# LuchnikovI/Differentiable-quantum-circuit-cuda

Hardware: AMD Instinct MI355X
Metric: gate-applications/sec (fwd+bwd) at n qubits (higher is better)
Workload: dtype c64 (f32)

## Files before the change

### differentiable-quantum-circuit-cuda_amd/csrc/qdc.hip

```cpp
#include "qdc_circuit.hpp"
#include "qdc_primitives.hpp"
#include "qdc_spec.hpp"

namespace {
template <int R>
struct SpecCheckTwo {
  __device__ __forceinline__ void operator()(qdc::cx (&xf)[R], qdc::cx (&xb)[R], const qdc::SpecEnv& E) const {
    constexpr uint32_t z[32] = {};
    qdc::spec_xchg_imm<6, false>(xf, E, z, z);
    qdc::spec_xchg<6, false>(xb, E, z, z, z, z);
  }
};
template <int R, int TB>
struct SpecCheckOne {
  __device__ __forceinline__ void operator()(qdc::cx (&x)[R], const qdc::SpecEnv& E) const {
    constexpr uint32_t z[32] = {};
    qdc::spec_xchg_imm<TB, true>(x, E, z, z);
    qdc::spec_xchg<TB, true>(x, E, z, z, z, z);
  }
};
}
#define QDC_SPEC_CHECK(name, threads, pass)                                                       \
  __global__ __launch_bounds__(threads) void name(qdc::chunk* f, qdc::chunk* b, const qdc::fop* ops, \
                                                  const qdc::cx* mats, qdc::fgeo fg, uint32_t l0,    \
// ... 455 lines not shown
  qdc::Plan p;
  if (!qdc::plan_lane(n, (int)R, pos2, pos1, 2048u, (reduces & 1) != 0, p, 1, (reduces & 2) ? 10u : 6u))
    return 1;
  const qdc::lgeo& g = p.lg;
  const unsigned v[10] = {(unsigned)(p.ampk + 1), g.nlow, g.nf, g.f0, g.f1, g.m0, g.m1,
                          (unsigned)(g.units & 0xffffffffu), (unsigned)(g.units >> 32), g.it};
  for (int i = 0; i < 10; ++i) out[i] = v[i];
  return 0;
}

static const char* spec_program_for(unsigned tile_bits, const unsigned* kinds, const unsigned* t1,
                                    const unsigned* t2, const unsigned long long* deps, size_t n,
                                    std::string& name, std::string& src) {
  if (n == 0 || n > 64) return "invalid arguments";
  std::vector<qdc::RqStage> st(n);
  for (size_t i = 0; i < n; ++i) st[i] = qdc::RqStage{kinds[i], t1[i], t2[i], deps ? deps[i] : 0};
  const bool force_one = (tile_bits & 0x100u) != 0, pf = (tile_bits & 0x200u) != 0;
  const bool spec_half = !(tile_bits & 0x400u);
  tile_bits &= 0xffu;
  const unsigned t2bits = sizeof(qdc::real) == 4 ? 11u : 10u;
  if (tile_bits != t2bits && tile_bits != t2bits + 1) return "tile_bits: not a specialized pass's tile";
  const bool two = tile_bits == t2bits && !force_one;
  qdc::RqKnobs knobs;
  if (tile_bits == t2bits && force_one) knobs.rq_wave |= pf ? 2 | 8 : 2;
  const qdc::RqVariant* V = qdc::rq_select(two, tile_bits, knobs, false);
  if (!V || !V->prefix) return "tile_bits: not a specialized pass's tile";
  const bool keep = spec_half && V->ns == 5;
  const qdc::RqPlan plan = qdc::rq_plan(st, tile_bits, nullptr, true, V->ns, keep);
  std::vector<qdc::SpecStep> sst;
  qdc::RqLayout cur = plan.load;
  for (const qdc::RqStep& s : plan.steps) {
    qdc::fop F{};
    if (s.relayout) {
      F.kind = qdc::FK_RELAYOUT;
      sst.push_back(qdc::SpecStep{true, cur, s.L, F});
      cur = s.L;
      continue;
    }
    F.kind = st[s.stage].kind | (two ? qdc::FOP_GAMMA : 0u);
    F.t1 = s.cs;
    const uint32_t kd = st[s.stage].kind;
    if ((kd == qdc::FK_Q2 || kd == qdc::FK_DIAG) && (s.cs >> 3) > (s.cs & 7u))
      F.t1 = (s.cs & 7u) * 8u + (s.cs >> 3);
    sst.push_back(qdc::SpecStep{false, cur, cur, F});
  }
  const bool half = V->pass_half && spec_half && !qdc::spec_imm() && qdc::spec_half_ok(sst);
  const qdc::SpecKind K = qdc::spec_kind(*V, half);
  const std::string body = qdc::spec_program_source(sst, tile_bits, K);
  name = qdc::spec_kernel_name(body, K);
  src = qdc::spec_kernel_source(name, body, K);
  return nullptr;
}

QDC_API const char* qdc_spec_selftest(unsigned tile_bits, const unsigned* kinds, const unsigned* t1,
// ... 240 lines not shown
```

### differentiable-quantum-circuit-cuda_amd/csrc/qdc_circuit.hpp

```cpp
#pragma once

#include <algorithm>
#include <cstring>
#include <memory>
#include <vector>

#include <rccl/rccl.h>

#include "qdc/circuit.h"
#include "qdc_device.hpp"
#include "qdc_shard.hpp"
#include "qdc_stage.hpp"
#include "qdc_fusion.hpp"
#include "qdc_jit.hpp"

namespace qdc {

struct Flat {
  const qdc_complex* data;
  std::vector<size_t> off;
  std::vector<size_t> len;
  Flat(const qdc_complex* d, const size_t* lens, size_t n) : data(d), off(n), len(n) {
    size_t o = 0;
    for (size_t i = 0; i < n; ++i) {
// ... 208 lines not shown
  int spec_async = sizeof(real) == 4 ? 1 : 0;
  std::map<std::vector<uint32_t>, SpecEntry> spec_cache;
  uint64_t spec_epoch = 0;
  int rq_permute = 1;
  int rq_perm_shard = 1;
  int rq_grad32 = 1;
  int rq_maxcl = 1;
  uint32_t rq_perm_low = 0;
  int rq_gstage = 1;
  uint32_t tile1_chunks = TILE_CHUNKS_1;
  int diag_inject = 1;
  int early_inject = 1;
  int dens1_kernel = 1;
  int dens_split = 1;
  int mirror = 1;
  int spec_half = 1;
  int defer_q1 = 1;
  bool mirror_on() const {
    return mirror && fuse && fuse_max_ops >= 2 && use_rq && (sizeof(real) == 4 || rq64);
  }
  const char* rq_variant(bool two, uint32_t tbits, const RqVariant*& V) const {
    V = rq_select(two, tbits, rqk, mirror_on());
    if (!V)
      return fail("no register-resident kernel for a %u-amplitude %s tile", 1u << tbits,
                  two ? "two-state" : "one-state");
    return nullptr;
  }
  bool rq_keep(const RqVariant& V) const { return spec_half && V.ns == 5; }

  bool dry = false;
  std::vector<unsigned char> dry_prog;
  std::vector<SpecEntry*> dry_specs;
  struct TraceOp {
    uint32_t dir, item, q2, q1, R, diag, mirrored, single;
    qdc_complex m[16];
  };
  bool tracing = false;
  std::vector<TraceOp> trace;
  size_t trace_from = 0;
  std::vector<uint8_t> inexact;
  uint32_t fused_blocks = 0;
  std::vector<std::pair<const void*, uint32_t>> fused_resident_cache;
  uint32_t last_fused_grid = 0;
  uint32_t last_fused_ndyn = 0;
  unsigned char* prog_host = nullptr;
  std::vector<StagePost> stage_post;
  size_t prog_cap = 0;

  Ctx& ctx0() { return devs[0]->ctx; }
  const char* sync_all() {
// ... 71 lines not shown
    if (const char* e = getenv("QDC_RW")) rqk.rq_wave = atoi(e);
    if (const char* e = getenv("QDC_RQ_ORDER")) rq_order = atoi(e);
    if (const char* e = getenv("QDC_RQ64")) rq64 = atoi(e);
    if (const char* e = getenv("QDC_RQ_SLOTS5")) rqk.rq_slots5 = atoi(e);
    if (const char* e = getenv("QDC_RQ_PERM")) rq_permute = atoi(e);
    if (const char* e = getenv("QDC_RQ_PERM_SHARD")) rq_perm_shard = atoi(e);
    if (const char* e = getenv("QDC_RQ_GRAD32")) rq_grad32 = atoi(e);
    if (const char* e = getenv("QDC_RQ_MAXCL")) rq_maxcl = atoi(e);
    if (const char* e = getenv("QDC_RQ_PERM_LOW")) rq_perm_low = (uint32_t)atoi(e);
    if (const char* e = getenv("QDC_RQ_GSTAGE")) rq_gstage = atoi(e);
    if (const char* e = getenv("QDC_DIAG_INJECT")) diag_inject = atoi(e);
    if (const char* e = getenv("QDC_EARLY_INJECT")) early_inject = atoi(e);
    if (const char* e = getenv("QDC_DENS1")) dens1_kernel = atoi(e);
    if (const char* e = getenv("QDC_DENS_SPLIT")) dens_split = atoi(e);
    if (const char* e = getenv("QDC_MIRROR")) mirror = atoi(e);
    if (const char* e = getenv("QDC_SPEC_HALF")) spec_half = atoi(e);
    if (const char* e = getenv("QDC_DEFER_Q1")) defer_q1 = atoi(e);
    if (const char* e = getenv("QDC_SCHED_CACHE")) sched_cache_on = atoi(e);
    if (const char* e = getenv("QDC_TILE1_CHUNKS")) {
      const uint32_t t = (uint32_t)atoi(e);
      if (t != TILE_CHUNKS_1 && t != TILE_CHUNKS_2)
        return fail("QDC_TILE1_CHUNKS must be %u or %u", TILE_CHUNKS_1, TILE_CHUNKS_2);
      tile1_chunks = t;
    }
    if (const char* e = getenv("QDC_SPEC")) spec_mode = atoi(e);
    if (const char* e = getenv("QDC_SPEC_MIN_QUBITS")) spec_min_qubits = (uint32_t)atoi(e);
    if (const char* e = getenv("QDC_SPEC_MAX")) spec_max = (uint32_t)atoi(e);
    if (const char* e = getenv("QDC_SPEC_FWD")) spec_fwd = atoi(e);
    if (const char* e = getenv("QDC_SPEC_ASYNC")) spec_async = atoi(e);
    SpecJit::get().set_processes(std::max(1, world / std::max(1, nlocal)));
// ... 692 lines not shown
      }
      g.diag = M.diag;
      g.role = stage_role(R, is_q1_gate(in.kind), op.pos2, lo, hi);
      const bool grad = two && is_var(in.kind);
      g.var = grad ? (int)B.var_idx[op.instr] : -1;
      any_grad = any_grad || grad;
    }
    SMat A;
    SMatD Bp;
    StagePost post;
    stage_compose(B.gates.data(), B.gates.size(), R, A, Bp, post);
    const bool all_diag = post.diag_only;
    if (rec_mats) (*rec_mats)[ii].push_back(A);
    SMat Aup = A;
    const bool from_fwd = B.backward && mirror_adjoint(B.plan, it, sj, R, Aup);
    if (tracing) {
      TraceOp t{B.backward ? 1u : 0u, (uint32_t)ii, hi, lo, (uint32_t)R, all_diag ? 1u : 0u,
                from_fwd ? 1u : 0u, 0u, {}};
      for (int i = 0; i < R * R; ++i) {
        const bool keep = !all_diag || i % (R + 1) == 0;
        t.m[i].re = keep ? (qdc_real)(real)Aup.a[i].real() : 0;
        t.m[i].im = keep ? (qdc_real)(real)Aup.a[i].imag() : 0;
      }
      trace.push_back(t);
    }
    fop& F = B.ops.back().F;
    F.t1 = local_bit(it, lo);
    F.t2 = local_bit(it, hi);
    F.mat = (uint32_t)B.mo;
    F.kind = (all_diag ? FK_DIAG : (R == 2 ? FK_Q1 : FK_Q2)) | (any_grad ? FOP_GAMMA : 0u);
    it.writes_f = true;
    const int nm = all_diag ? 4 : R * R;
    cx* m = B.mats + B.mo;
    for (int i = 0; i < nm; ++i) {
      const cd va = all_diag ? Aup.a[i * 4 + i] : Aup.a[i];
      const cdd vb = all_diag ? Bp.a[i * 4 + i] : Bp.a[i];
      m[i] = cx{(real)va.real(), (real)va.imag()};
      m[nm + i] = cx{(real)vb.real(), (real)vb.imag()};
    }
    B.mo += 2 * nm;
    const double cmac = all_diag ? 1.0 : (R == 2 ? 2.0 : 4.0);
    it.flops_per_amp += 8.0 * cmac * ((two ? 2.0 : 1.0) + (any_grad ? 1.0 : 0.0));
    if (any_grad) {
      post.slot = B.next_slot++;
      it.grad_slots.push_back(post.slot);
      B.ops.back().slot = (int)post.slot;
      it.has_red = true;
      stage_post.push_back(std::move(post));
    }
    return nullptr;
  }
  bool mirror_adjoint(const std::vector<qdc_plan_op>& plan, const Item& it, size_t sj, int R,
                      SMat& Aup) const {
    if (it.mirror_of.empty()) return false;
// ... 758 lines not shown
```

### differentiable-quantum-circuit-cuda_amd/csrc/qdc_jit.hpp

```cpp
#pragma once

#include <dirent.h>
#include <dlfcn.h>
#include <fcntl.h>
#include <spawn.h>
#include <sys/file.h>
#include <sys/stat.h>
#include <sys/wait.h>
#include <unistd.h>

#include <algorithm>
#include <atomic>
#include <chrono>
#include <cerrno>
#include <condition_variable>
#include <csignal>
#include <cstdlib>
#include <deque>
#include <ctime>
#include <cstdio>
#include <cstring>
#include <map>
#include <mutex>
#include <set>
// ... 128 lines not shown
    if (s.relayout) {
      const rq_layout c = rq_descriptor(s.Lc, T), n = rq_descriptor(s.Ln, T);
      b += "    { constexpr uint32_t rc[" + nr + "] = " + arr(c.rp, NR) + ", tc[8] = " + arr(c.tv, 8) +
           ", rn[" + nr + "] = " + arr(n.rp, NR) + ", tn[8] = " + arr(n.tv, 8) + ";\n      ";
      b += K.two ? "spec_xchg" + xt + "(xf, E, rc, tc, rn, tn); spec_xchg" + xt + "(xb, E, rc, tc, rn, tn); }\n"
                 : "spec_xchg" + xt + "(x, E, rc, tc, rn, tn); }\n";
      continue;
    }
    const uint32_t kind = s.F.kind & 7u;
    const bool gamma = K.two && (s.F.kind & FOP_GAMMA) != 0 && !(QDC_RQ_ABL & 4);
    const uint32_t c = s.F.t1;
    std::string tpl = kind == FK_Q1 ? "rq_q1<" + std::to_string(c)
                                    : std::string(kind == FK_DIAG ? "rq_diag<" : "rq_q2<") +
                                          std::to_string(c >> 3) + ", " + std::to_string(c & 7u);
    if (K.two)
      snprintf(tmp, sizeof tmp, "    %s, true, %u>(xf, xb, E.mats + E.ops[%zu].mat, %s, &E.accw[%u][0]);\n",
               tpl.c_str(), NR, j, gamma ? "true" : "false", ri);
    else
      snprintf(tmp, sizeof tmp, "    %s, false, %u>(x, x, E.mats + E.ops[%zu].mat, false, nullptr);\n",
               tpl.c_str(), NR, j);
    b += tmp;
    if (gamma) ++ri;
  }
  return b;
}
inline std::string spec_kernel_source(const std::string& name, const std::string& body, const SpecKind& K) {
  const std::string R = std::to_string(1u << K.ns);
  const std::string args =
      K.two ? "qdc::cx (&xf)[" + R + "], qdc::cx (&xb)[" + R + "], const qdc::SpecEnv& E"
            : "qdc::cx (&x)[" + R + "], const qdc::SpecEnv& E";
  return "#define QDC_SPEC_TU 1\n#include \"qdc_spec.hpp\"\n"
         "namespace {\n"
// ... 701 lines not shown
```

### differentiable-quantum-circuit-cuda_amd/csrc/qdc_kernels.hpp

```cpp
#pragma once

#include <cstddef>

#include <hip/hip_runtime.h>
#include <stdint.h>

#include <type_traits>

namespace qdc {

#ifdef QDC_F64
using real = double;
typedef double vec16 __attribute__((ext_vector_type(2)));
#else
using real = float;
typedef float vec16 __attribute__((ext_vector_type(4)));
#endif

struct cx {
  real x, y;
};

constexpr int VEC = 16 / (int)sizeof(cx);
constexpr int LV = (VEC == 2) ? 1 : 0;
// ... 971 lines not shown
#if QDC_PK_ASM
__device__ __forceinline__ pk2 pk_re_fma(pk2 a, pk2 f, pk2 c) {
  asm("v_pk_fma_f32 %0, %1, %2, %0 op_sel_hi:[0,1,1]" : "+v"(c) : "s"(a), "v"(f));
  return c;
}
__device__ __forceinline__ pk2 pk_im_fma(pk2 a, pk2 f, pk2 c) {
  asm("v_pk_fma_f32 %0, %1, %2, %0 op_sel:[1,1,0] op_sel_hi:[1,0,1] neg_lo:[1,0,0]"
      : "+v"(c) : "s"(a), "v"(f));
  return c;
}
__device__ __forceinline__ pk2 pk_re_mul(pk2 a, pk2 f) {
  pk2 r;
  asm("v_pk_mul_f32 %0, %1, %2 op_sel_hi:[0,1]" : "=v"(r) : "s"(a), "v"(f));
  return r;
}
#else
__device__ __forceinline__ pk2 pk_re_fma(pk2 a, pk2 f, pk2 c) {
  return __builtin_elementwise_fma(__builtin_shufflevector(a, a, 0, 0), f, c);
}
__device__ __forceinline__ pk2 pk_im_fma(pk2 a, pk2 f, pk2 c) {
  const pk2 na = -a;
  return __builtin_elementwise_fma(__builtin_shufflevector(na, a, 1, 3),
                                   __builtin_shufflevector(f, f, 1, 0), c);
}
__device__ __forceinline__ pk2 pk_re_mul(pk2 a, pk2 f) {
  return __builtin_shufflevector(a, a, 0, 0) * f;
}
#endif
#if QDC_PK_ASM || QDC_PK_VASM
__device__ __forceinline__ pk2 vpk_re_fma(pk2 a, pk2 f, pk2 c) {
  asm("v_pk_fma_f32 %0, %1, %2, %0 op_sel_hi:[0,1,1]" : "+v"(c) : "v"(a), "v"(f));
  return c;
}
__device__ __forceinline__ pk2 vpk_im_fma(pk2 a, pk2 f, pk2 c) {
  asm("v_pk_fma_f32 %0, %1, %2, %0 op_sel:[1,1,0] op_sel_hi:[1,0,1] neg_lo:[1,0,0]"
      : "+v"(c) : "v"(a), "v"(f));
  return c;
}
__device__ __forceinline__ pk2 vpk_re_mul(pk2 a, pk2 f) {
  pk2 r;
  asm("v_pk_mul_f32 %0, %1, %2 op_sel_hi:[0,1]" : "=v"(r) : "v"(a), "v"(f));
  return r;
}
#else
__device__ __forceinline__ pk2 vpk_re_fma(pk2 a, pk2 f, pk2 c) { return pk_re_fma(a, f, c); }
__device__ __forceinline__ pk2 vpk_im_fma(pk2 a, pk2 f, pk2 c) { return pk_im_fma(a, f, c); }
__device__ __forceinline__ pk2 vpk_re_mul(pk2 a, pk2 f) { return pk_re_mul(a, f); }
#endif
__device__ __forceinline__ cx ucfma(cx a, cx f, cx c) {
  const pk2 A = __builtin_bit_cast(pk2, a), F = __builtin_bit_cast(pk2, f);
  return __builtin_bit_cast(cx, pk_im_fma(A, F, pk_re_fma(A, F, __builtin_bit_cast(pk2, c))));
}
__device__ __forceinline__ cx ucmul(cx a, cx f) {
  const pk2 A = __builtin_bit_cast(pk2, a), F = __builtin_bit_cast(pk2, f);
  return __builtin_bit_cast(cx, pk_im_fma(A, F, pk_re_mul(A, F)));
}
__device__ __forceinline__ cx vcfma(cx a, cx f, cx c) {
  const pk2 A = __builtin_bit_cast(pk2, a), F = __builtin_bit_cast(pk2, f);
  return __builtin_bit_cast(cx, vpk_im_fma(A, F, vpk_re_fma(A, F, __builtin_bit_cast(pk2, c))));
}
__device__ __forceinline__ cx vcmul(cx a, cx f) {
  const pk2 A = __builtin_bit_cast(pk2, a), F = __builtin_bit_cast(pk2, f);
  return __builtin_bit_cast(cx, vpk_im_fma(A, F, vpk_re_mul(A, F)));
}
#else
__device__ __forceinline__ cx ucfma(cx a, cx f, cx c) { return cfma(a, f, c); }
__device__ __forceinline__ cx ucmul(cx a, cx f) { return cmul(a, f); }
__device__ __forceinline__ cx vcfma(cx a, cx f, cx c) { return cfma(a, f, c); }
__device__ __forceinline__ cx vcmul(cx a, cx f) { return cmul(a, f); }
#endif

template <int R>
__device__ __forceinline__ void umatvec(const cx* M, cx (&x)[R]) {
  cx y[R];
#pragma unroll
  for (int p = 0; p < R; ++p) {
    cx t = ucmul(M[p * R], x[0]);
#pragma unroll
    for (int q = 1; q < R; ++q) t = ucfma(M[p * R + q], x[q], t);
    y[p] = t;
  }
#pragma unroll
  for (int p = 0; p < R; ++p) x[p] = y[p];
}
// ... 13 lines not shown
      }
#pragma unroll
    for (int p = 0; p < R; ++p)
#pragma unroll
      for (int n = 0; n < NQ; ++n)
        y[n][p] = pk_im_fma(__builtin_bit_cast(pk2, M[p * R + q]), __builtin_bit_cast(pk2, x[n][q]),
                            y[n][p]);
  }
#pragma unroll
  for (int n = 0; n < NQ; ++n)
#pragma unroll
    for (int p = 0; p < R; ++p) x[n][p] = __builtin_bit_cast(cx, y[n][p]);
#else
#pragma unroll
  for (int n = 0; n < NQ; ++n) umatvec<R>(M, x[n]);
#endif
}

__device__ __forceinline__ uint32_t lane_sel(uint32_t f, uint32_t t, uint64_t mask) {
  uint32_t r;
  asm volatile("v_cndmask_b32_e64 %0, %1, %2, %3" : "=v"(r) : "v"(f), "v"(t), "s"(mask));
  return r;
}
__device__ __forceinline__ float lane_sel(float f, float t, uint64_t mask) {
  return __uint_as_float(lane_sel(__float_as_uint(f), __float_as_uint(t), mask));
}
__device__ __forceinline__ double lane_sel(double f, double t, uint64_t mask) {
  const uint64_t fb = (uint64_t)__double_as_longlong(f), tb = (uint64_t)__double_as_longlong(t);
  const uint64_t lo = lane_sel((uint32_t)fb, (uint32_t)tb, mask);
  const uint64_t hi = lane_sel((uint32_t)(fb >> 32), (uint32_t)(tb >> 32), mask);
// ... 123 lines not shown
__host__ __device__ __forceinline__ uint32_t swz(uint32_t i) {
  return i ^ (((i >> (4 + LV)) & 15u) << LV);
}
__device__ __forceinline__ uint32_t swz_chunk(uint32_t c) { return c ^ ((c >> 4) & 15u); }

enum : uint32_t {
  FK_Q1 = 0,
  FK_Q2 = 1,
  FK_DIAG = 2,
  FK_DENS1 = 3,
  FK_DENS2 = 4,
  FK_INJ1 = 5,
  FK_INJ2 = 6,
};
constexpr uint32_t FOP_GAMMA = 8;

#ifndef QDC_FUSED_WAVES
#define QDC_FUSED_WAVES 4
#endif
template <bool TWO, int TB, bool HASRED, bool WF, int NT>
__global__ __launch_bounds__(NT) __attribute__((amdgpu_waves_per_eu(NT == 256 ? QDC_FUSED_WAVES : 2)))
void k_fused(chunk* __restrict__ f, chunk* __restrict__ b, const fop* __restrict__ ops,
             const cx* __restrict__ mats, fgeo fg, cx* __restrict__ partials,
             uint64_t slot_stride) {
  constexpr int NS = TWO ? 2 : 1;
  constexpr int CPT = TB / NT;
  static_assert(TB % NT == 0 && TB * VEC >= 4 * NT, "tile must cover the block");
  __shared__ chunk lds[NS][TB];
  __shared__ real accw[HASRED ? NT / 64 : 1][HASRED ? FMAX_GRAD : 1][FACC];
  const uint32_t t = threadIdx.x;
// ... 529 lines not shown
```

### differentiable-quantum-circuit-cuda_amd/csrc/qdc_rq.hpp

```cpp
#pragma once

#include <type_traits>

#include "qdc_kernels.hpp"

namespace qdc {

#ifndef QDC_RQ_GSPLIT
#define QDC_RQ_GSPLIT 0
#endif
#ifndef QDC_MATVEC_N
#define QDC_MATVEC_N 1
#endif

constexpr int RQ_R = 16;
constexpr uint32_t FK_RELAYOUT = 7;
constexpr int RQ_NT_ONE = 256;
constexpr int RQ_NT_TWO = 128;

struct rq_layout {
  uint32_t rp[2 * RQ_R];
  uint32_t tv[8];
};
static_assert(sizeof(rq_layout) == 160 && sizeof(rq_layout) % sizeof(cx) == 0,
// ... 8 lines not shown
template <int S1, int S2>
__device__ __forceinline__ constexpr int rq_el(int base, int r) {
  return base | ((r & 1) << S1) | ((r >> 1) << S2);
}
template <int S1, int S2>
__device__ __forceinline__ constexpr int rq_base(int k) {
  int b = 0, bit = 0;
  for (int s = 0; s < 8; ++s) {
    if (s == S1 || s == S2) continue;
    if ((k >> bit) & 1) b |= 1 << s;
    ++bit;
  }
  return b;
}

template <int S1, int S2, bool TWO, int R>
__device__ __forceinline__ void rq_q2(cx (&f)[R], cx (&b)[R], const cx* __restrict__ M,
                                      bool gamma, real* acc_out) {
  cx A[16], B[16];
  if (TWO && gamma) {
    constexpr int NH = (QDC_RQ_GSPLIT && R >= 32) ? 2 : 1;
#pragma unroll
    for (int h = 0; h < NH; ++h) {
      constexpr int PR = 4 / NH;
      cx acc[4 * PR];
#pragma unroll
      for (int k = 0; k < R / 4; ++k) {
        const int base = rq_base<S1, S2>(k);
#pragma unroll
        for (int pp = 0; pp < PR; ++pp)
#pragma unroll
          for (int q = 0; q < 4; ++q) {
            const int p = h * PR + pp;
            const cx bp = b[rq_el<S1, S2>(base, p)], fq = f[rq_el<S1, S2>(base, q)];
            acc[pp * 4 + q] = k == 0 ? vcmul(bp, fq) : vcfma(bp, fq, acc[pp * 4 + q]);
          }
      }
      real v[8 * PR];
#pragma unroll
      for (int i = 0; i < 4 * PR; ++i) {
        v[2 * i] = acc[i].x;
        v[2 * i + 1] = acc[i].y;
      }
      wave_reduce_add<8 * PR>(v, acc_out + h * 8 * PR);
    }
  }
#pragma unroll
  for (int i = 0; i < 16; ++i) A[i] = M[i];
  constexpr int NQ = (QDC_MATVEC_N && R / 4 >= 2) ? 2 : 1;
#pragma unroll
  for (int k = 0; k < R / 4; k += NQ) {
    cx x[NQ][4];
#pragma unroll
    for (int n = 0; n < NQ; ++n)
#pragma unroll
      for (int r = 0; r < 4; ++r) x[n][r] = f[rq_el<S1, S2>(rq_base<S1, S2>(k + n), r)];
    umatvec_n<4, NQ>(A, x);
#pragma unroll
    for (int n = 0; n < NQ; ++n)
#pragma unroll
      for (int r = 0; r < 4; ++r) f[rq_el<S1, S2>(rq_base<S1, S2>(k + n), r)] = x[n][r];
  }
  if constexpr (TWO) {
#pragma unroll
// ... 2 lines not shown
    for (int k = 0; k < R / 4; k += NQ) {
      cx x[NQ][4];
#pragma unroll
      for (int n = 0; n < NQ; ++n)
#pragma unroll
        for (int r = 0; r < 4; ++r) x[n][r] = b[rq_el<S1, S2>(rq_base<S1, S2>(k + n), r)];
      umatvec_n<4, NQ>(B, x);
#pragma unroll
      for (int n = 0; n < NQ; ++n)
#pragma unroll
        for (int r = 0; r < 4; ++r) b[rq_el<S1, S2>(rq_base<S1, S2>(k + n), r)] = x[n][r];
    }
  }
}

template <int S1, int S2, bool TWO, int R>
__device__ __forceinline__ void rq_diag(cx (&f)[R], cx (&b)[R], const cx* __restrict__ M,
                                        bool gamma, real* acc_out) {
  cx A[4], B[4];
#pragma unroll
  for (int i = 0; i < 4; ++i) A[i] = M[i];
  if constexpr (TWO) {
#pragma unroll
    for (int i = 0; i < 4; ++i) B[i] = M[4 + i];
  }
  if (TWO && gamma) {
    cx acc[4];
#pragma unroll
    for (int k = 0; k < R / 4; ++k) {
      const int base = rq_base<S1, S2>(k);
#pragma unroll
      for (int r = 0; r < 4; ++r) {
        const int e = rq_el<S1, S2>(base, r);
        acc[r] = k == 0 ? vcmul(b[e], f[e]) : vcfma(b[e], f[e], acc[r]);
      }
    }
    real v[8];
#pragma unroll
    for (int i = 0; i < 4; ++i) {
      v[2 * i] = acc[i].x;
      v[2 * i + 1] = acc[i].y;
    }
    wave_reduce_add<8>(v, acc_out);
  }
#pragma unroll
  for (int k = 0; k < R / 4; ++k) {
    const int base = rq_base<S1, S2>(k);
#pragma unroll
    for (int r = 0; r < 4; ++r) {
      const int e = rq_el<S1, S2>(base, r);
      f[e] = ucmul(A[r], f[e]);
      if constexpr (TWO) b[e] = ucmul(B[r], b[e]);
    }
  }
}

template <int S, bool TWO, int R>
__device__ __forceinline__ void rq_q1(cx (&f)[R], cx (&b)[R], const cx* __restrict__ M,
                                      bool gamma, real* acc_out) {
  cx A[4], B[4];
#pragma unroll
  for (int i = 0; i < 4; ++i) A[i] = M[i];
  if constexpr (TWO) {
#pragma unroll
    for (int i = 0; i < 4; ++i) B[i] = M[4 + i];
  }
  constexpr int LOWM = (1 << S) - 1;
  if (TWO && gamma) {
    cx acc[4];
#pragma unroll
    for (int k = 0; k < R / 2; ++k) {
      const int j0 = ((k & ~LOWM) << 1) | (k & LOWM), j1 = j0 | (1 << S);
      const cx bx[2] = {b[j0], b[j1]}, fx[2] = {f[j0], f[j1]};
#pragma unroll
      for (int p = 0; p < 2; ++p)
#pragma unroll
        for (int q = 0; q < 2; ++q)
          acc[p * 2 + q] = k == 0 ? vcmul(bx[p], fx[q]) : vcfma(bx[p], fx[q], acc[p * 2 + q]);
    }
    real v[8];
#pragma unroll
    for (int i = 0; i < 4; ++i) {
      v[2 * i] = acc[i].x;
      v[2 * i + 1] = acc[i].y;
    }
    wave_reduce_add<8>(v, acc_out);
  }
  constexpr int NP = (QDC_MATVEC_N && R / 2 >= 4) ? 4 : 1;
#pragma unroll
  for (int k = 0; k < R / 2; k += NP) {
    cx x[NP][2];
#pragma unroll
    for (int n = 0; n < NP; ++n) {
      const int j0 = (((k + n) & ~LOWM) << 1) | ((k + n) & LOWM), j1 = j0 | (1 << S);
      x[n][0] = f[j0];
      x[n][1] = f[j1];
    }
    umatvec_n<2, NP>(A, x);
#pragma unroll
    for (int n = 0; n < NP; ++n) {
      const int j0 = (((k + n) & ~LOWM) << 1) | ((k + n) & LOWM), j1 = j0 | (1 << S);
      f[j0] = x[n][0];
      f[j1] = x[n][1];
    }
    if constexpr (TWO) {
#pragma unroll
      for (int n = 0; n < NP; ++n) {
        const int j0 = (((k + n) & ~LOWM) << 1) | ((k + n) & LOWM), j1 = j0 | (1 << S);
        x[n][0] = b[j0];
        x[n][1] = b[j1];
      }
      umatvec_n<2, NP>(B, x);
#pragma unroll
      for (int n = 0; n < NP; ++n) {
        const int j0 = (((k + n) & ~LOWM) << 1) | ((k + n) & LOWM), j1 = j0 | (1 << S);
        b[j0] = x[n][0];
        b[j1] = x[n][1];
      }
    }
  }
}

template <bool TWO, int R>
__device__ __forceinline__ void rq_stage(uint32_t sel, cx (&xf)[R], cx (&xb)[R],
                                         const cx* __restrict__ M, bool gamma, real* acc) {
#define QDC_RQ_Q2(S1, S2)                                                             \
  case FK_Q2 * 64 + (S1) * 8 + (S2):                                                  \
    if constexpr ((S2) < 4 || R >= 32) rq_q2<S1, S2, TWO, R>(xf, xb, M, gamma, acc);   \
    break;                                                                            \
  case FK_DIAG * 64 + (S1) * 8 + (S2):                                                \
    if constexpr ((S2) < 4 || R >= 32) rq_diag<S1, S2, TWO, R>(xf, xb, M, gamma, acc); \
    break;
  switch (sel) {
    QDC_RQ_Q2(0, 1) QDC_RQ_Q2(0, 2) QDC_RQ_Q2(0, 3) QDC_RQ_Q2(1, 2) QDC_RQ_Q2(1, 3)
    QDC_RQ_Q2(2, 3) QDC_RQ_Q2(0, 4) QDC_RQ_Q2(1, 4) QDC_RQ_Q2(2, 4) QDC_RQ_Q2(3, 4)
    case FK_Q1 * 64 + 0: rq_q1<0, TWO, R>(xf, xb, M, gamma, acc); break;
    case FK_Q1 * 64 + 1: rq_q1<1, TWO, R>(xf, xb, M, gamma, acc); break;
    case FK_Q1 * 64 + 2: rq_q1<2, TWO, R>(xf, xb, M, gamma, acc); break;
    case FK_Q1 * 64 + 4:
      if constexpr (R >= 32) rq_q1<4, TWO, R>(xf, xb, M, gamma, acc);
      break;
    default: rq_q1<3, TWO, R>(xf, xb, M, gamma, acc); break;
  }
#undef QDC_RQ_Q2
}

template <int LOGNT>
__device__ __forceinline__ uint32_t rq_tp(const rq_layout* L, uint32_t t) {
  uint32_t tp = 0;
#pragma unroll
  for (int k = 0; k < LOGNT; ++k) tp ^= ((t >> k) & 1u) ? L->tv[k] : 0u;
  return tp;
}

__device__ __forceinline__ void rq_exchange(cx (&x)[RQ_R], cx* buf, uint32_t tp,
                                            const rq_layout* Lc, uint32_t tpn,
                                            const rq_layout* Ln) {
#if !(QDC_RQ_ABL & 16)
  __syncthreads();
// ... 241 lines not shown
      }
      if ((QDC_RQ_ABL & 1) && kind != FK_RELAYOUT) {
        if (TWO && (op.kind & FOP_GAMMA)) ++ri;
        continue;
      }
      if (kind == FK_RELAYOUT) {
        const rq_layout* Lc = reinterpret_cast<const rq_layout*>(mats + lcur);
        const rq_layout* Ln = reinterpret_cast<const rq_layout*>(M);
        const uint32_t tp = TWO ? rq_tp<LOGNT>(Lc, t) : tpc, tpn = rq_tp<LOGNT>(Ln, t);
        rq_exchange(xf, buf, tp, Lc, tpn, Ln);
        if constexpr (TWO) rq_exchange(xb, buf, tp, Lc, tpn, Ln);
        tpc = tpn;
        lcur = op.mat;
        continue;
      }
      rq_stage<TWO>(kind * 64u + op.t1, xf, xb, M, gamma, acc);
      if (gamma) ++ri;
    }
  };
  if constexpr (!PF) {
    cx xf[RQ_R], xb[RQ_R];
    for (uint32_t tt = 0; tt < count; ++tt) {
      const uint64_t base = tile_base(tile0 + tt * tstep);
      load(xf, xb, base);
      run(xf, xb);
      store(xf, xb, base);
    }
  } else {
    static_assert(!TWO, "k_rq prefetch: one-state passes (qdc_variant.hpp)");
    constexpr int NLD = TWO ? 2 * CPT : CPT;
    vec16 pf_f[CPT];
// ... 254 lines not shown
        continue;
      }
      if ((QDC_RQ_ABL & 1) && kind != FK_RELAYOUT) {
        if (TWO && (op.kind & FOP_GAMMA)) ++ri;
        continue;
      }
      if (kind == FK_RELAYOUT) {
        const rq_layout* Lc = reinterpret_cast<const rq_layout*>(mats + lcur);
        const rq_layout* Ln = reinterpret_cast<const rq_layout*>(M);
        const uint32_t tp = rq_tp<TB>(Lc, lane), tpn = rq_tp<TB>(Ln, lane);
        exchange(xf, tp, Lc, tpn, Ln);
        if constexpr (TWO) exchange(xb, tp, Lc, tpn, Ln);
        lcur = op.mat;
        continue;
      }
      rq_stage<TWO>(kind * 64u + op.t1, xf, xb, M, gamma, acc);
      if (gamma) ++ri;
    }
  };
  auto flush_acc = [&](cx* dst, uint64_t stride) __attribute__((always_inline)) {
    __builtin_amdgcn_wave_barrier();
    for (uint32_t i = lane; i < fg.ngrad * FACC; i += 64) {
      const uint32_t k = i / FACC, e = i % FACC;
      reinterpret_cast<real*>(dst + (uint64_t)k * stride)[e] = accw[k][e];
      accw[k][e] = 0;
    }
    __builtin_amdgcn_wave_barrier();
  };
  cx xf[R], xb[R];
  if constexpr (!PF) {
    if (QDC_RQ_ABL & 32) {
// ... 182 lines not shown
```

### differentiable-quantum-circuit-cuda_amd/quantum_differentiable_circuit/__init__.py

```python
from __future__ import annotations

import ctypes as C
from typing import List, Sequence

import numpy as np

from .common_gates import get_cnot, get_hadamard
from ._native import (PanicException, KernelStat, PlanOp, check, default_precision, load,
                      ptr, PRECISIONS)
from .observable import PauliSum

__all__ = ["Circuit", "Circuit32", "Circuit64", "QuantizedTensor", "PanicException",
           "get_q1_grad", "get_q2_grad", "get_q2_grad_diag", "get_qk_grad", "data_transfer",
           "PauliSum", "pauli_inject",
           "circuit_class",
           "plan", "unpermute", "get_hadamard", "get_cnot"]

(CONST_Q2, VAR_Q2, CONST_Q2_NONU, VAR_Q2_NONU, CONST_Q2_DIAG, VAR_Q2_DIAG, CONST_Q1,
 CONST_Q1_NONU, VAR_Q1, VAR_Q1_NONU, Q2_DENSITY, Q1_DENSITY, DIFF_Q2_DENSITY,
 DIFF_Q1_DENSITY) = range(14)
MODE_RUN, MODE_FORWARD = 0, 1


def _array1(x, dtype, what):
# ... 414 lines not shown
    dens = [_array2(g, dt, "grads_wrt_density") for g in grads_wrt_density]
    df, dl = _flatten(dens, dt, "grads_wrt_density", "Gradient is not contiguous.")
    count = C.c_size_t(0)
    check(lib.qdc_precompile(int(qubits_number), int(world), kinds, a, b, m, ptr(cf), ptr(cl),
                             len(const_gates), ptr(vf), ptr(vl), len(var_gates), ptr(df), ptr(dl),
                             len(dens), C.byref(count)))
    return int(count.value)


def trace_program(qubits_number, instructions, const_gates, var_gates, grads_wrt_density,
                  world=1, precision=None):
    prec = precision or default_precision()
    lib = load(prec)
    dt = np.dtype(PRECISIONS[prec])
    rec = np.dtype([("dir", "<u4"), ("item", "<u4"), ("q2", "<u4"), ("q1", "<u4"), ("R", "<u4"),
                    ("diag", "<u4"), ("mirrored", "<u4"), ("single", "<u4"), ("m", dt, 16)])
    m = len(instructions)
    kinds = (C.c_int * m)(*[int(i[0]) for i in instructions])
    a = (C.c_uint * m)(*[int(i[1]) for i in instructions])
    b = (C.c_uint * m)(*[int(i[2]) if len(i) > 2 else 0 for i in instructions])
    cf, cl = _flat_gates(const_gates, dt, "const_gates")
    vf, vl = _flat_gates(var_gates, dt, "var_gates")
    dens = [_array2(g, dt, "grads_wrt_density") for g in grads_wrt_density]
    df, dl = _flatten(dens, dt, "grads_wrt_density", "Gradient is not contiguous.")
    cap = 4 * m + 64
    while True:
        out = np.zeros(cap, dtype=rec)
        cnt = C.c_size_t(0)
        check(lib.qdc_trace_program(int(qubits_number), int(world), kinds, a, b, m, ptr(cf),
                                    ptr(cl), len(const_gates), ptr(vf), ptr(vl), len(var_gates),
                                    ptr(df), ptr(dl), len(dens), ptr(out), cap, C.byref(cnt)))
# ... 245 lines not shown
```

### include/qdc/circuit.h

```cpp
#ifndef QDC_CIRCUIT_H
#define QDC_CIRCUIT_H

#include <stddef.h>

#include "qdc/primitives.h"

#ifdef __cplusplus
extern "C" {
#endif

enum qdc_kind {
  QDC_CONST_Q2 = 0,
  QDC_VAR_Q2 = 1,
  QDC_CONST_Q2_NONU = 2,
  QDC_VAR_Q2_NONU = 3,
  QDC_CONST_Q2_DIAG = 4,
  QDC_VAR_Q2_DIAG = 5,
  QDC_CONST_Q1 = 6,
  QDC_CONST_Q1_NONU = 7,
  QDC_VAR_Q1 = 8,
  QDC_VAR_Q1_NONU = 9,
  QDC_Q2_DENSITY = 10,
  QDC_Q1_DENSITY = 11,
  QDC_DIFF_Q2_DENSITY = 12,
// ... 122 lines not shown

const char* qdc_precompile(size_t qubits_number, int world, const int* kinds,
                           const unsigned* pos2, const unsigned* pos1, size_t count,
                           const qdc_complex* const_gates, const size_t* const_lens, size_t n_const,
                           const qdc_complex* var_gates, const size_t* var_lens, size_t n_var,
                           const qdc_complex* dens_grads, const size_t* dens_lens, size_t n_dens,
                           size_t* kernels);

const char* qdc_check_schedule(size_t qubits_number, int world, const int* kinds,
                               const unsigned* pos2, const unsigned* pos1, size_t count,
                               size_t* items, size_t* swaps);

typedef struct qdc_trace_op {
  unsigned dir, item, q2, q1, R, diag, mirrored, single;
  qdc_complex m[16];
} qdc_trace_op;

const char* qdc_trace_program(size_t qubits_number, int world, const int* kinds,
                              const unsigned* pos2, const unsigned* pos1, size_t count,
                              const qdc_complex* const_gates, const size_t* const_lens,
                              size_t n_const, const qdc_complex* var_gates,
                              const size_t* var_lens, size_t n_var, const qdc_complex* dens_grads,
                              const size_t* dens_lens, size_t n_dens, qdc_trace_op* out, size_t cap,
                              size_t* n_out);

#ifdef __cplusplus
}
#endif

#endif
// ... 1 lines not shown
```

Baseline: 4790.

## Derive backward-state gate matrix as conjugate of forward matrix in register kernels

For backward-pass fused gates whose instructions are unitary and exactly representable, the second (b) matrix is now set to the elementwise conjugate of the forward matrix. The register-resident kernels then load only the A matrix and apply it to both the forward and backward amplitudes, using packed FMA variants that negate the imaginary part. This saves matrix loads and registers. Matrix fetches are also moved ahead of the gradient reduction, with a scheduling barrier, so their latency overlaps that work; a LATE flag keeps the old fetch order when the feature is disabled. The trace format grows to expose the b matrices. The risks are extra kernel template variants and a correctness dependence on the conjugate identity holding.

```diff
diff --git a/differentiable-quantum-circuit-cuda_amd/csrc/qdc.hip b/differentiable-quantum-circuit-cuda_amd/csrc/qdc.hip
--- a/differentiable-quantum-circuit-cuda_amd/csrc/qdc.hip
+++ b/differentiable-quantum-circuit-cuda_amd/csrc/qdc.hip
@@ -493,7 +493,8 @@
                                     std::string& name, std::string& src) {
   if (n == 0 || n > 64) return "invalid arguments";
   std::vector<qdc::RqStage> st(n);
-  for (size_t i = 0; i < n; ++i) st[i] = qdc::RqStage{kinds[i], t1[i], t2[i], deps ? deps[i] : 0};
+  for (size_t i = 0; i < n; ++i)
+    st[i] = qdc::RqStage{kinds[i] & 7u, t1[i], t2[i], deps ? deps[i] : 0};
   const bool force_one = (tile_bits & 0x100u) != 0, pf = (tile_bits & 0x200u) != 0;
   const bool spec_half = !(tile_bits & 0x400u);
   tile_bits &= 0xffu;
@@ -516,7 +517,7 @@
       cur = s.L;
       continue;
     }
-    F.kind = st[s.stage].kind | (two ? qdc::FOP_GAMMA : 0u);
+    F.kind = st[s.stage].kind | (two ? qdc::FOP_GAMMA | (kinds[s.stage] & qdc::FOP_CONJB) : 0u);
     F.t1 = s.cs;
     const uint32_t kd = st[s.stage].kind;
     if ((kd == qdc::FK_Q2 || kd == qdc::FK_DIAG) && (s.cs >> 3) > (s.cs & 7u))
diff --git a/differentiable-quantum-circuit-cuda_amd/csrc/qdc_circuit.hpp b/differentiable-quantum-circuit-cuda_amd/csrc/qdc_circuit.hpp
--- a/differentiable-quantum-circuit-cuda_amd/csrc/qdc_circuit.hpp
+++ b/differentiable-quantum-circuit-cuda_amd/csrc/qdc_circuit.hpp
@@ -246,6 +246,7 @@
   int dens1_kernel = 1;
   int dens_split = 1;
   int mirror = 1;
+  int conjb = 1;
   int spec_half = 1;
   int defer_q1 = 1;
   bool mirror_on() const {
@@ -266,6 +267,8 @@
   struct TraceOp {
     uint32_t dir, item, q2, q1, R, diag, mirrored, single;
     qdc_complex m[16];
+    qdc_complex b[16];
+    uint32_t conjb, reserved;
   };
   bool tracing = false;
   std::vector<TraceOp> trace;
@@ -367,6 +370,7 @@
     if (const char* e = getenv("QDC_DENS1")) dens1_kernel = atoi(e);
     if (const char* e = getenv("QDC_DENS_SPLIT")) dens_split = atoi(e);
     if (const char* e = getenv("QDC_MIRROR")) mirror = atoi(e);
+    if (const char* e = getenv("QDC_CONJB")) conjb = atoi(e);
     if (const char* e = getenv("QDC_SPEC_HALF")) spec_half = atoi(e);
     if (const char* e = getenv("QDC_DEFER_Q1")) defer_q1 = atoi(e);
     if (const char* e = getenv("QDC_SCHED_CACHE")) sched_cache_on = atoi(e);
@@ -1089,30 +1093,39 @@
     if (rec_mats) (*rec_mats)[ii].push_back(A);
     SMat Aup = A;
     const bool from_fwd = B.backward && mirror_adjoint(B.plan, it, sj, R, Aup);
-    if (tracing) {
-      TraceOp t{B.backward ? 1u : 0u, (uint32_t)ii, hi, lo, (uint32_t)R, all_diag ? 1u : 0u,
-                from_fwd ? 1u : 0u, 0u, {}};
-      for (int i = 0; i < R * R; ++i) {
-        const bool keep = !all_diag || i % (R + 1) == 0;
-        t.m[i].re = keep ? (qdc_real)(real)Aup.a[i].real() : 0;
-        t.m[i].im = keep ? (qdc_real)(real)Aup.a[i].imag() : 0;
-      }
-      trace.push_back(t);
-    }
-    fop& F = B.ops.back().F;
-    F.t1 = local_bit(it, lo);
-    F.t2 = local_bit(it, hi);
-    F.mat = (uint32_t)B.mo;
-    F.kind = (all_diag ? FK_DIAG : (R == 2 ? FK_Q1 : FK_Q2)) | (any_grad ? FOP_GAMMA : 0u);
-    it.writes_f = true;
+    bool cj = B.backward && conjb != 0;
+    for (uint32_t pi : st) {
+      const uint32_t k = B.plan[pi].instr;
+      cj = cj && !is_nonu(ins[k].kind) && !(k < inexact.size() && inexact[k]);
+    }
     const int nm = all_diag ? 4 : R * R;
     cx* m = B.mats + B.mo;
     for (int i = 0; i < nm; ++i) {
       const cd va = all_diag ? Aup.a[i * 4 + i] : Aup.a[i];
       const cdd vb = all_diag ? Bp.a[i * 4 + i] : Bp.a[i];
       m[i] = cx{(real)va.real(), (real)va.imag()};
-      m[nm + i] = cx{(real)vb.real(), (real)vb.imag()};
-    }
+      m[nm + i] = cj ? cx{m[i].x, -m[i].y} : cx{(real)vb.real(), (real)vb.imag()};
+    }
+    if (tracing) {
+      TraceOp t{B.backward ? 1u : 0u, (uint32_t)ii, hi, lo, (uint32_t)R, all_diag ? 1u : 0u,
+                from_fwd ? 1u : 0u, 0u, {}, {}, cj ? 1u : 0u, 0u};
+      for (int i = 0; i < R * R; ++i) {
+        const bool keep = !all_diag || i % (R + 1) == 0;
+        t.m[i].re = keep ? (qdc_real)(real)Aup.a[i].real() : 0;
+        t.m[i].im = keep ? (qdc_real)(real)Aup.a[i].imag() : 0;
+        const cx vb = all_diag ? m[nm + i / (R + 1)] : m[nm + i];
+        t.b[i].re = keep ? (qdc_real)vb.x : 0;
+        t.b[i].im = keep ? (qdc_real)vb.y : 0;
+      }
+      trace.push_back(t);
+    }
+    fop& F = B.ops.back().F;
+    F.t1 = local_bit(it, lo);
+    F.t2 = local_bit(it, hi);
+    F.mat = (uint32_t)B.mo;
+    F.kind = (all_diag ? FK_DIAG : (R == 2 ? FK_Q1 : FK_Q2)) | (any_grad ? FOP_GAMMA : 0u) |
+             (cj ? FOP_CONJB : 0u) | (conjb == 0 ? FOP_LATE : 0u);
+    it.writes_f = true;
     B.mo += 2 * nm;
     const double cmac = all_diag ? 1.0 : (R == 2 ? 2.0 : 4.0);
     it.flops_per_amp += 8.0 * cmac * ((two ? 2.0 : 1.0) + (any_grad ? 1.0 : 0.0));
diff --git a/differentiable-quantum-circuit-cuda_amd/csrc/qdc_jit.hpp b/differentiable-quantum-circuit-cuda_amd/csrc/qdc_jit.hpp
--- a/differentiable-quantum-circuit-cuda_amd/csrc/qdc_jit.hpp
+++ b/differentiable-quantum-circuit-cuda_amd/csrc/qdc_jit.hpp
@@ -166,8 +166,9 @@
                                     : std::string(kind == FK_DIAG ? "rq_diag<" : "rq_q2<") +
                                           std::to_string(c >> 3) + ", " + std::to_string(c & 7u);
     if (K.two)
-      snprintf(tmp, sizeof tmp, "    %s, true, %u>(xf, xb, E.mats + E.ops[%zu].mat, %s, &E.accw[%u][0]);\n",
-               tpl.c_str(), NR, j, gamma ? "true" : "false", ri);
+      snprintf(tmp, sizeof tmp, "    %s, true, %u%s>(xf, xb, E.mats + E.ops[%zu].mat, %s, &E.accw[%u][0]%s);\n",
+               tpl.c_str(), NR, (s.F.kind & FOP_CONJB) ? ", true" : "", j, gamma ? "true" : "false", ri,
+               (s.F.kind & FOP_LATE) ? ", true" : "");
     else
       snprintf(tmp, sizeof tmp, "    %s, false, %u>(x, x, E.mats + E.ops[%zu].mat, false, nullptr);\n",
                tpl.c_str(), NR, j);
diff --git a/differentiable-quantum-circuit-cuda_amd/csrc/qdc_kernels.hpp b/differentiable-quantum-circuit-cuda_amd/csrc/qdc_kernels.hpp
--- a/differentiable-quantum-circuit-cuda_amd/csrc/qdc_kernels.hpp
+++ b/differentiable-quantum-circuit-cuda_amd/csrc/qdc_kernels.hpp
@@ -1009,6 +1009,11 @@
   asm("v_pk_mul_f32 %0, %1, %2 op_sel_hi:[0,1]" : "=v"(r) : "s"(a), "v"(f));
   return r;
 }
+__device__ __forceinline__ pk2 pk_imc_fma(pk2 a, pk2 f, pk2 c) {
+  asm("v_pk_fma_f32 %0, %1, %2, %0 op_sel:[1,1,0] op_sel_hi:[1,0,1] neg_hi:[1,0,0]"
+      : "+v"(c) : "s"(a), "v"(f));
+  return c;
+}
 #else
 __device__ __forceinline__ pk2 pk_re_fma(pk2 a, pk2 f, pk2 c) {
   return __builtin_elementwise_fma(__builtin_shufflevector(a, a, 0, 0), f, c);
@@ -1021,6 +1026,11 @@
 __device__ __forceinline__ pk2 pk_re_mul(pk2 a, pk2 f) {
   return __builtin_shufflevector(a, a, 0, 0) * f;
 }
+__device__ __forceinline__ pk2 pk_imc_fma(pk2 a, pk2 f, pk2 c) {
+  const pk2 na = -a;
+  return __builtin_elementwise_fma(__builtin_shufflevector(a, na, 1, 3),
+                                   __builtin_shufflevector(f, f, 1, 0), c);
+}
 #endif
 #if QDC_PK_ASM || QDC_PK_VASM
 __device__ __forceinline__ pk2 vpk_re_fma(pk2 a, pk2 f, pk2 c) {
@@ -1050,6 +1060,10 @@
   const pk2 A = __builtin_bit_cast(pk2, a), F = __builtin_bit_cast(pk2, f);
   return __builtin_bit_cast(cx, pk_im_fma(A, F, pk_re_mul(A, F)));
 }
+__device__ __forceinline__ cx ucmulc(cx a, cx f) {
+  const pk2 A = __builtin_bit_cast(pk2, a), F = __builtin_bit_cast(pk2, f);
+  return __builtin_bit_cast(cx, pk_imc_fma(A, F, pk_re_mul(A, F)));
+}
 __device__ __forceinline__ cx vcfma(cx a, cx f, cx c) {
   const pk2 A = __builtin_bit_cast(pk2, a), F = __builtin_bit_cast(pk2, f);
   return __builtin_bit_cast(cx, vpk_im_fma(A, F, vpk_re_fma(A, F, __builtin_bit_cast(pk2, c))));
@@ -1060,9 +1074,13 @@
 }
 #else
 __device__ __forceinline__ cx ucfma(cx a, cx f, cx c) { return cfma(a, f, c); }
-__device__ __forceinline__ cx ucmul(cx a, cx f) { return cmul(a, f); }
+__device__ __forceinline__ cx cmul_fixed(cx a, cx b) {
+  return {fma(a.x, b.x, -(a.y * b.y)), fma(a.x, b.y, a.y * b.x)};
+}
+__device__ __forceinline__ cx ucmul(cx a, cx f) { return cmul_fixed(a, f); }
+__device__ __forceinline__ cx ucmulc(cx a, cx f) { return cmul_fixed(cx{a.x, -a.y}, f); }
 __device__ __forceinline__ cx vcfma(cx a, cx f, cx c) { return cfma(a, f, c); }
-__device__ __forceinline__ cx vcmul(cx a, cx f) { return cmul(a, f); }
+__device__ __forceinline__ cx vcmul(cx a, cx f) { return cmul_fixed(a, f); }
 #endif
 
 template <int R>
@@ -1106,6 +1124,49 @@
 #else
 #pragma unroll
   for (int n = 0; n < NQ; ++n) umatvec<R>(M, x[n]);
+#endif
+}
+
+template <int R, int NQ>
+__device__ __forceinline__ void umatvec_nc(const cx* M, cx (&x)[NQ][R], cx (&z)[NQ][R]) {
+#ifndef QDC_F64
+  pk2 y[NQ][R], w[NQ][R];
+#pragma unroll
+  for (int q = 0; q < R; ++q) {
+#pragma unroll
+    for (int p = 0; p < R; ++p)
+#pragma unroll
+      for (int n = 0; n < NQ; ++n) {
+        const pk2 a = __builtin_bit_cast(pk2, M[p * R + q]);
+        const pk2 f = __builtin_bit_cast(pk2, x[n][q]), g = __builtin_bit_cast(pk2, z[n][q]);
+        y[n][p] = q == 0 ? pk_re_mul(a, f) : pk_re_fma(a, f, y[n][p]);
+        w[n][p] = q == 0 ? pk_re_mul(a, g) : pk_re_fma(a, g, w[n][p]);
+      }
+#pragma unroll
+    for (int p = 0; p < R; ++p)
+#pragma unroll
+      for (int n = 0; n < NQ; ++n) {
+        const pk2 a = __builtin_bit_cast(pk2, M[p * R + q]);
+        y[n][p] = pk_im_fma(a, __builtin_bit_cast(pk2, x[n][q]), y[n][p]);
+        w[n][p] = pk_imc_fma(a, __builtin_bit_cast(pk2, z[n][q]), w[n][p]);
+      }
+  }
+#pragma unroll
+  for (int n = 0; n < NQ; ++n)
+#pragma unroll
+    for (int p = 0; p < R; ++p) {
+      x[n][p] = __builtin_bit_cast(cx, y[n][p]);
+      z[n][p] = __builtin_bit_cast(cx, w[n][p]);
+    }
+#else
+  cx C[R * R];
+#pragma unroll
+  for (int i = 0; i < R * R; ++i) C[i] = cx{M[i].x, -M[i].y};
+#pragma unroll
+  for (int n = 0; n < NQ; ++n) {
+    umatvec<R>(M, x[n]);
+    umatvec<R>(C, z[n]);
+  }
 #endif
 }
 
@@ -1259,6 +1320,8 @@
   FK_INJ2 = 6,
 };
 constexpr uint32_t FOP_GAMMA = 8;
+constexpr uint32_t FOP_CONJB = 16;
+constexpr uint32_t FOP_LATE = 32;
 
 #ifndef QDC_FUSED_WAVES
 #define QDC_FUSED_WAVES 4
diff --git a/differentiable-quantum-circuit-cuda_amd/csrc/qdc_rq.hpp b/differentiable-quantum-circuit-cuda_amd/csrc/qdc_rq.hpp
--- a/differentiable-quantum-circuit-cuda_amd/csrc/qdc_rq.hpp
+++ b/differentiable-quantum-circuit-cuda_amd/csrc/qdc_rq.hpp
@@ -46,10 +46,19 @@
   return b;
 }
 
-template <int S1, int S2, bool TWO, int R>
+template <int N>
+__device__ __forceinline__ void rq_fetch(cx (&A)[N], const cx* __restrict__ M, bool pin) {
+#pragma unroll
+  for (int i = 0; i < N; ++i) A[i] = M[i];
+  if (pin) __builtin_amdgcn_sched_barrier(0);
+}
+
+template <int S1, int S2, bool TWO, int R, bool CJ = false>
 __device__ __forceinline__ void rq_q2(cx (&f)[R], cx (&b)[R], const cx* __restrict__ M,
-                                      bool gamma, real* acc_out) {
+                                      bool gamma, real* acc_out, bool late = false) {
   cx A[16], B[16];
+  const bool ahead = !(TWO && gamma && late);
+  if (ahead) rq_fetch(A, M, TWO && gamma);
   if (TWO && gamma) {
     constexpr int NH = (QDC_RQ_GSPLIT && R >= 32) ? 2 : 1;
 #pragma unroll
@@ -77,9 +86,30 @@
       wave_reduce_add<8 * PR>(v, acc_out + h * 8 * PR);
     }
   }
-#pragma unroll
-  for (int i = 0; i < 16; ++i) A[i] = M[i];
+  if (!ahead) rq_fetch(A, M, false);
   constexpr int NQ = (QDC_MATVEC_N && R / 4 >= 2) ? 2 : 1;
+  if constexpr (TWO && CJ) {
+#pragma unroll
+    for (int k = 0; k < R / 4; k += NQ) {
+      cx x[NQ][4], z[NQ][4];
+#pragma unroll
+      for (int n = 0; n < NQ; ++n)
+#pragma unroll
+        for (int r = 0; r < 4; ++r) {
+          x[n][r] = f[rq_el<S1, S2>(rq_base<S1, S2>(k + n), r)];
+          z[n][r] = b[rq_el<S1, S2>(rq_base<S1, S2>(k + n), r)];
+        }
+      umatvec_nc<4, NQ>(A, x, z);
+#pragma unroll
+      for (int n = 0; n < NQ; ++n)
+#pragma unroll
+        for (int r = 0; r < 4; ++r) {
+          f[rq_el<S1, S2>(rq_base<S1, S2>(k + n), r)] = x[n][r];
+          b[rq_el<S1, S2>(rq_base<S1, S2>(k + n), r)] = z[n][r];
+        }
+    }
+    return;
+  }
 #pragma unroll
   for (int k = 0; k < R / 4; k += NQ) {
     cx x[NQ][4];
@@ -112,16 +142,25 @@
   }
 }
 
-template <int S1, int S2, bool TWO, int R>
+template <int S1, int S2, bool TWO, int R, bool CJ = false>
 __device__ __forceinline__ void rq_diag(cx (&f)[R], cx (&b)[R], const cx* __restrict__ M,
-                                        bool gamma, real* acc_out) {
+                                        bool gamma, real* acc_out, bool late = false) {
   cx A[4], B[4];
-#pragma unroll
-  for (int i = 0; i < 4; ++i) A[i] = M[i];
-  if constexpr (TWO) {
-#pragma unroll
-    for (int i = 0; i < 4; ++i) B[i] = M[4 + i];
-  }
+  auto fetch = [&](bool pin) __attribute__((always_inline)) {
+    if constexpr (TWO && !CJ) {
+      cx AB[8];
+      rq_fetch(AB, M, pin);
+#pragma unroll
+      for (int i = 0; i < 4; ++i) {
+        A[i] = AB[i];
+        B[i] = AB[4 + i];
+      }
+    } else {
+      rq_fetch(A, M, pin);
+    }
+  };
+  const bool ahead = !(TWO && gamma && late);
+  if (ahead) fetch(TWO && gamma);
   if (TWO && gamma) {
     cx acc[4];
 #pragma unroll
@@ -141,6 +180,7 @@
     }
     wave_reduce_add<8>(v, acc_out);
   }
+  if (!ahead) fetch(false);
 #pragma unroll
   for (int k = 0; k < R / 4; ++k) {
     const int base = rq_base<S1, S2>(k);
@@ -148,21 +188,30 @@
     for (int r = 0; r < 4; ++r) {
       const int e = rq_el<S1, S2>(base, r);
       f[e] = ucmul(A[r], f[e]);
-      if constexpr (TWO) b[e] = ucmul(B[r], b[e]);
-    }
-  }
-}
-
-template <int S, bool TWO, int R>
+      if constexpr (TWO) b[e] = CJ ? ucmulc(A[r], b[e]) : ucmul(B[r], b[e]);
+    }
+  }
+}
+
+template <int S, bool TWO, int R, bool CJ = false>
 __device__ __forceinline__ void rq_q1(cx (&f)[R], cx (&b)[R], const cx* __restrict__ M,
-                                      bool gamma, real* acc_out) {
+                                      bool gamma, real* acc_out, bool late = false) {
   cx A[4], B[4];
-#pragma unroll
-  for (int i = 0; i < 4; ++i) A[i] = M[i];
-  if constexpr (TWO) {
-#pragma unroll
-    for (int i = 0; i < 4; ++i) B[i] = M[4 + i];
-  }
+  auto fetch = [&](bool pin) __attribute__((always_inline)) {
+    if constexpr (TWO && !CJ) {
+      cx AB[8];
+      rq_fetch(AB, M, pin);
+#pragma unroll
+      for (int i = 0; i < 4; ++i) {
+        A[i] = AB[i];
+        B[i] = AB[4 + i];
+      }
+    } else {
+      rq_fetch(A, M, pin);
+    }
+  };
+  const bool ahead = !(TWO && gamma && late);
+  if (ahead) fetch(TWO && gamma);
   constexpr int LOWM = (1 << S) - 1;
   if (TWO && gamma) {
     cx acc[4];
@@ -184,63 +233,69 @@
     }
     wave_reduce_add<8>(v, acc_out);
   }
+  if (!ahead) fetch(false);
   constexpr int NP = (QDC_MATVEC_N && R / 2 >= 4) ? 4 : 1;
 #pragma unroll
   for (int k = 0; k < R / 2; k += NP) {
-    cx x[NP][2];
+    cx x[NP][2], z[NP][2];
 #pragma unroll
     for (int n = 0; n < NP; ++n) {
       const int j0 = (((k + n) & ~LOWM) << 1) | ((k + n) & LOWM), j1 = j0 | (1 << S);
       x[n][0] = f[j0];
       x[n][1] = f[j1];
-    }
-    umatvec_n<2, NP>(A, x);
+      if constexpr (TWO) {
+        z[n][0] = b[j0];
+        z[n][1] = b[j1];
+      }
+    }
+    if constexpr (TWO && CJ) {
+      umatvec_nc<2, NP>(A, x, z);
+    } else {
+      umatvec_n<2, NP>(A, x);
+      if constexpr (TWO) umatvec_n<2, NP>(B, z);
+    }
 #pragma unroll
     for (int n = 0; n < NP; ++n) {
       const int j0 = (((k + n) & ~LOWM) << 1) | ((k + n) & LOWM), j1 = j0 | (1 << S);
       f[j0] = x[n][0];
       f[j1] = x[n][1];
-    }
-    if constexpr (TWO) {
-#pragma unroll
-      for (int n = 0; n < NP; ++n) {
-        const int j0 = (((k + n) & ~LOWM) << 1) | ((k + n) & LOWM), j1 = j0 | (1 << S);
-        x[n][0] = b[j0];
-        x[n][1] = b[j1];
-      }
-      umatvec_n<2, NP>(B, x);
-#pragma unroll
-      for (int n = 0; n < NP; ++n) {
-        const int j0 = (((k + n) & ~LOWM) << 1) | ((k + n) & LOWM), j1 = j0 | (1 << S);
-        b[j0] = x[n][0];
-        b[j1] = x[n][1];
+      if constexpr (TWO) {
+        b[j0] = z[n][0];
+        b[j1] = z[n][1];
       }
     }
   }
 }
 
 template <bool TWO, int R>
-__device__ __forceinline__ void rq_stage(uint32_t sel, cx (&xf)[R], cx (&xb)[R],
+__device__ __forceinline__ void rq_stage(uint32_t sel, uint32_t fl, cx (&xf)[R], cx (&xb)[R],
                                          const cx* __restrict__ M, bool gamma, real* acc) {
-#define QDC_RQ_Q2(S1, S2)                                                             \
-  case FK_Q2 * 64 + (S1) * 8 + (S2):                                                  \
-    if constexpr ((S2) < 4 || R >= 32) rq_q2<S1, S2, TWO, R>(xf, xb, M, gamma, acc);   \
-    break;                                                                            \
-  case FK_DIAG * 64 + (S1) * 8 + (S2):                                                \
-    if constexpr ((S2) < 4 || R >= 32) rq_diag<S1, S2, TWO, R>(xf, xb, M, gamma, acc); \
+  const bool cj = (fl & FOP_CONJB) != 0, late = (fl & FOP_LATE) != 0;
+#define QDC_RQ_CJ(FN, ...)                                         \
+  do {                                                             \
+    if (TWO && cj) FN<__VA_ARGS__, TWO, R, TWO>(xf, xb, M, gamma, acc, late); \
+    else FN<__VA_ARGS__, TWO, R, false>(xf, xb, M, gamma, acc, late);    \
+  } while (0)
+#define QDC_RQ_Q2(S1, S2)                                         \
+  case FK_Q2 * 64 + (S1) * 8 + (S2):                              \
+    if constexpr ((S2) < 4 || R >= 32) QDC_RQ_CJ(rq_q2, S1, S2);   \
+    break;                                                        \
+  case FK_DIAG * 64 + (S1) * 8 + (S2):                            \
+    if constexpr ((S2) < 4 || R >= 32) QDC_RQ_CJ(rq_diag, S1, S2); \
     break;
   switch (sel) {
     QDC_RQ_Q2(0, 1) QDC_RQ_Q2(0, 2) QDC_RQ_Q2(0, 3) QDC_RQ_Q2(1, 2) QDC_RQ_Q2(1, 3)
     QDC_RQ_Q2(2, 3) QDC_RQ_Q2(0, 4) QDC_RQ_Q2(1, 4) QDC_RQ_Q2(2, 4) QDC_RQ_Q2(3, 4)
-    case FK_Q1 * 64 + 0: rq_q1<0, TWO, R>(xf, xb, M, gamma, acc); break;
-    case FK_Q1 * 64 + 1: rq_q1<1, TWO, R>(xf, xb, M, gamma, acc); break;
-    case FK_Q1 * 64 + 2: rq_q1<2, TWO, R>(xf, xb, M, gamma, acc); break;
+    case FK_Q1 * 64 + 0: QDC_RQ_CJ(rq_q1, 0); break;
+    case FK_Q1 * 64 + 1: QDC_RQ_CJ(rq_q1, 1); break;
+    case FK_Q1 * 64 + 2: QDC_RQ_CJ(rq_q1, 2); break;
     case FK_Q1 * 64 + 4:
-      if constexpr (R >= 32) rq_q1<4, TWO, R>(xf, xb, M, gamma, acc);
+      if constexpr (R >= 32) QDC_RQ_CJ(rq_q1, 4);
       break;
-    default: rq_q1<3, TWO, R>(xf, xb, M, gamma, acc); break;
+    default: QDC_RQ_CJ(rq_q1, 3); break;
   }
 #undef QDC_RQ_Q2
+#undef QDC_RQ_CJ
 }
 
 template <int LOGNT>
@@ -512,7 +567,7 @@
         lcur = op.mat;
         continue;
       }
-      rq_stage<TWO>(kind * 64u + op.t1, xf, xb, M, gamma, acc);
+      rq_stage<TWO>(kind * 64u + op.t1, op.kind, xf, xb, M, gamma, acc);
       if (gamma) ++ri;
     }
   };
@@ -797,7 +852,7 @@
         lcur = op.mat;
         continue;
       }
-      rq_stage<TWO>(kind * 64u + op.t1, xf, xb, M, gamma, acc);
+      rq_stage<TWO>(kind * 64u + op.t1, op.kind, xf, xb, M, gamma, acc);
       if (gamma) ++ri;
     }
   };
diff --git a/differentiable-quantum-circuit-cuda_amd/quantum_differentiable_circuit/__init__.py b/differentiable-quantum-circuit-cuda_amd/quantum_differentiable_circuit/__init__.py
--- a/differentiable-quantum-circuit-cuda_amd/quantum_differentiable_circuit/__init__.py
+++ b/differentiable-quantum-circuit-cuda_amd/quantum_differentiable_circuit/__init__.py
@@ -452,7 +452,8 @@
     lib = load(prec)
     dt = np.dtype(PRECISIONS[prec])
     rec = np.dtype([("dir", "<u4"), ("item", "<u4"), ("q2", "<u4"), ("q1", "<u4"), ("R", "<u4"),
-                    ("diag", "<u4"), ("mirrored", "<u4"), ("single", "<u4"), ("m", dt, 16)])
+                    ("diag", "<u4"), ("mirrored", "<u4"), ("single", "<u4"), ("m", dt, 16),
+                    ("b", dt, 16), ("conjb", "<u4"), ("reserved", "<u4")])
     m = len(instructions)
     kinds = (C.c_int * m)(*[int(i[0]) for i in instructions])
     a = (C.c_uint * m)(*[int(i[1]) for i in instructions])
diff --git a/include/qdc/circuit.h b/include/qdc/circuit.h
--- a/include/qdc/circuit.h
+++ b/include/qdc/circuit.h
@@ -160,6 +160,8 @@
 typedef struct qdc_trace_op {
   unsigned dir, item, q2, q1, R, diag, mirrored, single;
   qdc_complex m[16];
+  qdc_complex b[16];
+  unsigned conjb, reserved;
 } qdc_trace_op;
 
 const char* qdc_trace_program(size_t qubits_number, int world, const int* kinds,
```

New measurement: 4809 (median of 4 runs). Within noise of the previous version (+0.4%).
